# guanlongzhao/fac-via-ppg

Measured on AMD Instinct MI355X. Metric: 22.05 kHz audio samples/sec end-to-end PPG→wav; real-time factor at batch=1, higher is better.
Workload: dtype f32

## Files before the change

fac-via-ppg_amd/csrc/facppg_gemm.hip:

```cpp
#include "facppg_gemm.h"

namespace facppg {
namespace {

constexpr int TN = 64, KCH = 64;

__global__ void k_pack_a(const float* __restrict__ src, float4* __restrict__ dst, int M, int Cin, int taps, int KG, long sm,
                         long sc, long st, long off) {
  const int idx = blockIdx.x * blockDim.x + threadIdx.x;
  const int MB = (M + 31) / 32;
  if (idx >= MB * (KG + 1) * 64) return;
  const int lane = idx & 63, g = (idx >> 6) % (KG + 1), mb = (idx >> 6) / (KG + 1);
  const int m = mb * 32 + (lane & 31), K = Cin * taps;
  float v[4];
  for (int s = 0; s < 4; ++s) {
    const int k = 8 * g + 4 * (lane >> 5) + s;
    const int tap = k / Cin, c = k - tap * Cin;
    v[s] = (m < M && k < K && g < KG) ? src[off + m * sm + c * sc + tap * st] : 0.0f;
  }
  dst[idx] = make_float4(v[0], v[1], v[2], v[3]);
}

struct KArgs {
  GemmArgs g;
  int KG;
  int sk;
};

__device__ __forceinline__ void gemm_epilogue(const GemmArgs& p, int b, int m, int n, float v) {
  if (p.bias) v += p.bias[m];
  if (p.scale) v = v * p.scale[m] + p.shift[m];
  if (p.act == ACT_RELU) v = fmaxf(v, 0.0f);
  else if (p.act == ACT_TANH) v = tanhf(v);
  else if (p.act == ACT_LOG_CLAMP) v = logf(fmaxf(v, 1e-5f));
  if (p.mask) v = v * (float)p.mask[(size_t)b * p.mask_bs + (size_t)m * p.ldmask + n] * 2.0f;
  if (p.res) v += p.res[(size_t)b * p.res_bs + (size_t)m * p.ldres + n];
  if (p.gate_ts) {
    const float T = p.gate_ts[(size_t)b * p.gate_bs + (size_t)m * p.ldgate + n];
    const float S = p.gate_ts[(size_t)b * p.gate_bs + (size_t)(p.M + m) * p.ldgate + n];
    p.C[(size_t)b * p.c_bs + (size_t)m * p.ldc + n] = v * S * (1.0f - T * T);
    p.C[(size_t)b * p.c_bs + (size_t)(p.M + m) * p.ldc + n] = v * T * S * (1.0f - S);
  } else if (p.c_transposed) p.C[(size_t)b * p.c_bs + (size_t)n * p.ldc + m] = v;
  else p.C[(size_t)b * p.c_bs + (size_t)m * p.ldc + n] = v;
}

__global__ __launch_bounds__(256) void k_gemm(KArgs ka) {
  const GemmArgs& p = ka.g;
  __shared__ __attribute__((aligned(16))) float smem[2 * KCH * TN];
  const int tid = threadIdx.x, lane = tid & 63, w = tid >> 6, li = lane & 31, kh = lane >> 5;
  const int b = blockIdx.z / ka.sk, ks = blockIdx.z % ka.sk, n0 = p.col0 + blockIdx.x * TN;
  const int Nb = p.n_valid ? min(p.N, p.n_valid[b] * p.n_valid_mul + p.n_valid_add) : p.N;
  if (n0 >= Nb) return;
  if (p.skip && *p.skip) return;
  const int Ns = p.src_hi > 0 ? (p.n_valid ? min(p.src_hi, p.n_valid[b] * p.n_valid_mul + p.n_valid_add) : p.src_hi) : Nb;
  const int mb = blockIdx.y * 4 + w;
  const int MB = (p.M + 31) / 32;
  const bool active = mb < MB;
  const int K = p.Cin * p.taps;
  const int nch_all = ka.KG / 8;
  const int c_lo = ks * nch_all / ka.sk, c_hi = (ks + 1) * nch_all / ka.sk;

  f32x16 acc[2];
#pragma unroll
  for (int r = 0; r < 16; ++r) { acc[0][r] = 0.0f; acc[1][r] = 0.0f; }

  const float* xb = p.X + (size_t)b * p.x_bs;
  const int col = n0 + lane;
  float stg[16];
  auto stage_load = [&](int c) {
#pragma unroll
    for (int j = 0; j < 16; ++j) {
      const int kk = c * KCH + w * 16 + j;
      const int tap = kk / p.Cin, ch = kk - tap * p.Cin;
      const int sc = col + (tap - p.pad) * p.dil;
      stg[j] = (kk < K && sc >= 0 && sc < Ns) ? xb[(size_t)ch * p.ldx + sc] : 0.0f;
    }
  };
  auto stage_write = [&](int buf) {
    float* dst = smem + buf * (KCH * TN) + (w * 16) * TN + lane;
#pragma unroll
    for (int j = 0; j < 16; ++j) dst[j * TN] = stg[j];
  };

  const float4* ap = p.A + (size_t)(active ? mb : 0) * (ka.KG + 1) * 64 + lane;
  constexpr int RING = 4;
  float4 ar[RING];
  stage_load(c_lo);
#pragma unroll
  for (int i = 0; i < RING - 1; ++i) ar[i] = ap[(size_t)(c_lo * 8 + i) * 64];
  stage_write(c_lo & 1);
  __syncthreads();
  for (int c = c_lo; c < c_hi; ++c) {
    stage_load(c + 1 < c_hi ? c + 1 : c);
    const float* lb = smem + (c & 1) * (KCH * TN) + (4 * kh) * TN + li;
    const int G = c * 8;
#pragma unroll
    for (int g = 0; g < 8; ++g) {
      ar[(g + RING - 1) % RING] = ap[(size_t)(G + g + RING - 1) * 64];
      __builtin_amdgcn_sched_barrier(0);
      const float4 a0 = ar[g % RING];
#pragma unroll
      for (int s = 0; s < 4; ++s) {
        const float av = s == 0 ? a0.x : s == 1 ? a0.y : s == 2 ? a0.z : a0.w;
        acc[0] = mfma32x32x2(av, lb[(8 * g + s) * TN], acc[0]);
        acc[1] = mfma32x32x2(av, lb[(8 * g + s) * TN + 32], acc[1]);
      }
    }
    stage_write((c + 1) & 1);
    __syncthreads();
  }
  if (!active) return;
#pragma unroll
  for (int cb = 0; cb < 2; ++cb) {
    const int n = n0 + cb * 32 + li;
    if (n >= Nb) continue;
#pragma unroll
    for (int r = 0; r < 16; ++r) {
      const int m = mb * 32 + 8 * (r >> 2) + (r & 3) + 4 * kh;
      if (m >= p.M) continue;
      if (ka.sk > 1) p.splitk_ws[(((size_t)ks * p.B + b) * p.M + m) * p.N + n] = acc[cb][r];
      else gemm_epilogue(p, b, m, n, acc[cb][r]);
    }
  }
}

__global__ void k_gemm_reduce(KArgs ka) {
  const GemmArgs& p = ka.g;
  const int n = p.col0 + blockIdx.x * blockDim.x + threadIdx.x, m = blockIdx.y, b = blockIdx.z;
  const int Nb = p.n_valid ? min(p.N, p.n_valid[b] * p.n_valid_mul + p.n_valid_add) : p.N;
  if (n >= Nb) return;
  if (p.skip && *p.skip) return;
  float v = 0.0f;
  for (int ks = 0; ks < ka.sk; ++ks) v += p.splitk_ws[(((size_t)ks * p.B + b) * p.M + m) * p.N + n];
  gemm_epilogue(p, b, m, n, v);
}

}

int pack_a_strided(const float* src, int M, int Cin, int taps, long sm, long sc, long st, long off, float4* dst, hipStream_t s) {
  const int KG = gemm_kpad(Cin * taps) / 8;
  const int total = (round_up(M, 32) / 32) * (KG + 1) * 64;
  k_pack_a<<<(total + 255) / 256, 256, 0, s>>>(src, dst, M, Cin, taps, KG, sm, sc, st, off);
  FACPPG_HIP_CHECK(hipGetLastError());
  return FACPPG_OK;
}

int pack_a(const float* src, int M, int Cin, int taps, float4* dst, hipStream_t s) {
  return pack_a_strided(src, M, Cin, taps, (long)Cin * taps, taps, 1, 0, dst, s);
}

int gemm_launch(const GemmArgs& a, hipStream_t s) {
  FACPPG_REQUIRE(a.A && a.X && a.C && a.M > 0 && a.N > 0 && a.Cin > 0 && a.taps > 0 && a.B > 0 && a.col0 >= 0 && a.col0 < a.N, FACPPG_EINVAL,
                 "gemm_launch: bad arguments");
  KArgs ka;
  ka.g = a;
  ka.KG = gemm_kpad(a.Cin * a.taps) / 8;
  ka.sk = 1;
  dim3 grid((a.N - a.col0 + TN - 1) / TN, (round_up(a.M, 32) / 32 + 3) / 4, a.B);
  const int nch = ka.KG / 8;
  if (a.splitk_ws && nch >= 8) {
    const int sk = nch / 4 < 16 ? nch / 4 : 16;
    const size_t need = (size_t)sk * a.B * a.M * a.N * sizeof(float);
    FACPPG_REQUIRE(need <= a.splitk_ws_bytes, FACPPG_EWORKSPACE, "gemm_launch: split-K buffer has %zu bytes, needs %zu",
                   a.splitk_ws_bytes, need);
    ka.sk = sk;
  }
  grid.z = a.B * ka.sk;
  k_gemm<<<grid, 256, 0, s>>>(ka);
  if (ka.sk > 1) k_gemm_reduce<<<dim3((a.N - a.col0 + 255) / 256, a.M, a.B), 256, 0, s>>>(ka);
  FACPPG_HIP_CHECK(hipGetLastError());
  return FACPPG_OK;
}

}
```

fac-via-ppg_amd/csrc/facppg_taco.hip:

```cpp

#include <algorithm>
#include <cstdlib>
#include <cstring>
#include <mutex>
#include <new>

#include "facppg_gemm.h"

using namespace facppg;

struct facppg_taco {
  facppg_taco_config c;
  int device;
  int coop_limit;
  int wall_khz;
  char* arena;
  float4 *pre0, *pre1, *conv[8], *wih;
  float *conv_b[8], *conv_scale[8], *conv_shift[8];
  float *whh_t[2], *lstm_b;
  float4* mem_w;
  float *dp0_t, *dp1_t, *att_t, *att_b, *dec_t, *dec_b, *q_t, *proj_t, *proj_b;
  float *loc_conv, *loc_dense, *v;
  float *att_coop[5], *dec_coop[5];
  int coop_U[5], coop_nwg[5];
// ... 102 lines not shown
  const int slot = tid % ns, ks = tid / ns;
  if (ks >= KS) return;
  const int k0 = (int)((long)ks * K / KS), k1 = (int)((long)(ks + 1) * K / KS);
  const float4* w = reinterpret_cast<const float4*>(WT) + slot;
  float4 acc = make_float4(0.f, 0.f, 0.f, 0.f);
  for (int kb = k0; kb < k1; kb += UB) {
    float4 wv[UB];
#pragma unroll
    for (int u = 0; u < UB; ++u) wv[u] = w[(size_t)min(kb + u, k1 - 1) * ns];
#pragma unroll
    for (int u = 0; u < UB; ++u) {
      const float vk = kb + u < k1 ? v[kb + u] : 0.0f;
      acc.x = fmaf(wv[u].x, vk, acc.x); acc.y = fmaf(wv[u].y, vk, acc.y);
      acc.z = fmaf(wv[u].z, vk, acc.z); acc.w = fmaf(wv[u].w, vk, acc.w);
    }
  }
  reinterpret_cast<float4*>(part)[ks * ns + slot] = acc;
}
template <int NT>
__device__ __forceinline__ int pick_ks(int Rp, int K) {
  int ks = NT / (Rp >> 2);
  if (ks > K) ks = K;
  return ks < 1 ? 1 : ks;
}
__device__ __forceinline__ float part_sum(const float* part, int Rp, int KS, int r) {
  float s = 0.0f;
#pragma unroll 8
  for (int i = 0; i < KS; ++i) s += part[i * Rp + r];
  return s;
}

__global__ __launch_bounds__(NT) void k_bilstm(const float* __restrict__ xproj, const float* __restrict__ whh_t0,
                                               const float* __restrict__ whh_t1, const int* __restrict__ lengths, int Tin, int H,
                                               float* __restrict__ mem_tm , float* __restrict__ mem_cm ) {
  extern __shared__ float sm[];
  const int dir = blockIdx.x, b = blockIdx.y, tid = threadIdx.x;
  const int R = 4 * H;
  float* hv = sm;
  float* cv = hv + H;
  float* part = cv + H;
  const float* WT = dir ? whh_t1 : whh_t0;
  const int len = lengths ? lengths[b] : Tin;
  const int KS = pick_ks<NT>(R, H);
  for (int i = tid; i < H; i += NT) { hv[i] = 0.0f; cv[i] = 0.0f; }
  __syncthreads();
  for (int s = 0; s < len; ++s) {
    const int t = dir ? len - 1 - s : s;
    matvec_part(WT, H, R, KS, hv, part, tid);
    __syncthreads();
    if (tid < H) {
      const float* xp = xproj + ((size_t)b * Tin + t) * (2 * R) + dir * R;
      const float gi = part_sum(part, R, KS, tid) + xp[tid];
      const float gf = part_sum(part, R, KS, H + tid) + xp[H + tid];
      const float gg = part_sum(part, R, KS, 2 * H + tid) + xp[2 * H + tid];
      const float go = part_sum(part, R, KS, 3 * H + tid) + xp[3 * H + tid];
      const float c = sigm(gf) * cv[tid] + sigm(gi) * tanhf(gg);
      const float h = sigm(go) * tanhf(c);
      cv[tid] = c; hv[tid] = h;
      mem_tm[((size_t)b * Tin + t) * (2 * H) + dir * H + tid] = h;
      mem_cm[((size_t)b * 2 * H + dir * H + tid) * Tin + t] = h;
    }
    __syncthreads();
  }
}

__constant__ unsigned long long g_poll_limit_ticks = 0;
__device__ __forceinline__ unsigned long long poll_tag(const unsigned long long* w, unsigned tag) {
  unsigned long long v;
  const unsigned long long limit = g_poll_limit_ticks;
  unsigned long long t0 = 0;
  unsigned spins = 0;
#pragma unroll 1
  do {
    v = __hip_atomic_load(w, __ATOMIC_RELAXED, __HIP_MEMORY_SCOPE_AGENT);
    if ((++spins & 1023u) == 0 && limit) {
      const unsigned long long now = wall_clock64();
      if (!t0) t0 = now;
      else if (now - t0 > limit) __builtin_trap();
    }
  } while ((unsigned)(v >> 32) != tag);
  return v;
}

template <int BU, int BKR>
__global__ __launch_bounds__(NTC) void k_bilstm_coop(const float* __restrict__ xproj, const float* __restrict__ whh_t0,
                                                     const float* __restrict__ whh_t1, const int* __restrict__ lengths, int Tin,
                                                     int H, unsigned long long* __restrict__ xchg ,
                                                     float* __restrict__ mem_tm, float* __restrict__ mem_cm) {
  constexpr int BKP = NTC / (4 * BU);
  __shared__ float hv[BKP * BKR];
  __shared__ float part[BKP][4 * BU];
  __shared__ float gates[4 * BU];
  const int wg = blockIdx.x, dir = blockIdx.y, b = blockIdx.z, tid = threadIdx.x;
  const int R = 4 * H, KR = (H + BKP - 1) / BKP;
  const int r = tid % (4 * BU), kp = tid / (4 * BU);
  const int u = wg * BU + r % BU, row = (r / BU) * H + u;
  const float* WT = dir ? whh_t1 : whh_t0;
  const int len = lengths ? lengths[b] : Tin;
  float w[BKR];
#pragma unroll
  for (int i = 0; i < BKR; ++i) {
    const int k = kp * KR + i;
    w[i] = (i < KR && k < H && u < H) ? WT[(size_t)k * R + row] : 0.0f;
  }
  for (int i = tid; i < BKP * BKR; i += NTC) hv[i] = 0.0f;
  float c = 0.0f;
  unsigned long long* xb = xchg + (size_t)(b * 2 + dir) * 2 * H;
  __syncthreads();
  for (int s = 0; s < len; ++s) {
    const int t = dir ? len - 1 - s : s;
    const float xp = (kp == 0 && u < H) ? xproj[((size_t)b * Tin + t) * (2 * R) + dir * R + row] : 0.0f;
    float acc = 0.0f;
    const float* hk = hv + kp * KR;
#pragma unroll
    for (int i = 0; i < BKR; ++i) acc = fmaf(w[i], hk[i], acc);
    part[kp][r] = acc;
    __syncthreads();
    if (kp == 0) {
      float g = xp;
#pragma unroll
      for (int j = 0; j < BKP; ++j) g += part[j][r];
      gates[r] = g;
    }
    __syncthreads();
    if (tid < BU && wg * BU + tid < H) {
      const float cn = sigm(gates[BU + tid]) * c + sigm(gates[tid]) * tanhf(gates[2 * BU + tid]);
      const float h = sigm(gates[3 * BU + tid]) * tanhf(cn);
      c = cn;
      const int uu = wg * BU + tid;
      __hip_atomic_store(xb + (size_t)((s + 1) & 1) * H + uu, ((unsigned long long)(unsigned)(s + 1) << 32) | __float_as_uint(h),
                         __ATOMIC_RELAXED, __HIP_MEMORY_SCOPE_AGENT);
      mem_tm[((size_t)b * Tin + t) * (2 * H) + dir * H + uu] = h;
      mem_cm[((size_t)b * 2 * H + dir * H + uu) * Tin + t] = h;
    }
    if (s + 1 < len) {
      const unsigned long long* src = xb + (size_t)((s + 1) & 1) * H;
      for (int i = tid; i < H; i += NTC) {
        hv[i] = __uint_as_float((unsigned)poll_tag(src + i, (unsigned)(s + 1)));
      }
    }
    __syncthreads();
  }
}

struct DecArgs {
  const float *dp0_t, *dp1_t, *att_t, *att_b, *dec_t, *dec_b, *q_t, *proj_t, *proj_b, *loc_conv, *loc_dense, *v;
  const float *att_coop, *dec_coop;
  unsigned long long* xchg;
  const float *att_w4, *dec_w4;
  const float *w1p_t, *b1p;
  unsigned long long* xsplit;
  long long* prof;
  const float* memory;
  const float* pm;
  const int* lengths;
  const int* step_limits;
  const uint8_t* masks;
  float* mel;
  float* gate;
  float* align;
  int* out_len;
  int B, Tin, E, P, A, D, AD, NF, NFIL, KSZ, window, max_steps, U;
  int b0;
  float gate_thr;
  int nwk, dbg_flags;
  unsigned long long* melx;
};

__device__ __forceinline__ int dec_step_limit(const DecArgs& p, int b) {
  return p.step_limits ? min(max(p.step_limits[b], 1), p.max_steps) : p.max_steps;
}

struct DecLds {
  float *in_att, *in_dec, *in_proj, *ac, *dc, *xin, *p1, *pq, *part, *feat, *lconv, *ldense, *vv, *wprev, *wcum, *en;
  int KA, KD, KP, ADp, NFp, Pp, G, AD32;
};

__host__ __device__ inline size_t dec_lds_floats(int P, int E, int A, int D, int NF, int AD, int NFIL, int KSZ, int Tin) {
  (void)NFIL;
  const size_t ADp32 = round_up(AD, 32);
  return (size_t)(P + E + A) + (A + E + D) + (D + E) + A + D + round_up(NF, 4) + round_up(P, 4) + ADp32 + 4096 +
         64 * 32 + (size_t)round_up(2 * KSZ, 2) * 32 + 32 * ADp32 + ADp32 + 3 * (size_t)Tin;
}

__device__ __forceinline__ void dec_carve(const DecArgs& p, float* sm, DecLds& L) {
  L.G = 4 * p.A;
  L.KA = p.P + p.E + p.A;
  L.KD = p.A + p.E + p.D;
  L.KP = p.D + p.E;
  L.ADp = round_up(p.AD, 4); L.NFp = round_up(p.NF + 1, 4); L.Pp = round_up(p.P, 4);
  L.AD32 = round_up(p.AD, 32);
  L.in_att = sm;
  L.in_dec = L.in_att + L.KA;
  L.in_proj = L.in_dec + L.KD;
  L.ac = L.in_proj + L.KP;
  L.dc = L.ac + p.A;
  L.xin = L.dc + p.D;
  L.p1 = L.xin + round_up(p.NF, 4);
  L.pq = L.p1 + L.Pp;
  L.part = L.pq + L.AD32;
  L.feat = L.part + 4096;
  L.lconv = L.feat + 64 * 32;
  L.ldense = L.lconv + round_up(2 * p.KSZ, 2) * 32;
  L.vv = L.ldense + 32 * L.AD32;
  L.wprev = L.vv + L.AD32;
  L.wcum = L.wprev + p.Tin;
  L.en = L.wcum + p.Tin;
}

template <int NT>
__device__ __forceinline__ void dec_init(const DecArgs& p, const DecLds& L, float* sm, int tid) {
  for (int i = tid; i < L.KA + L.KD + L.KP + p.A + p.D + round_up(p.NF, 4) + L.Pp + L.AD32; i += NT) sm[i] = 0.0f;
  const int KK = 2 * p.KSZ;
  for (int i = tid; i < round_up(KK, 2) * 32; i += NT) {
    const int kk = i >> 5, f = i & 31;
    L.lconv[i] = (kk < KK && f < p.NFIL) ? p.loc_conv[f * KK + kk] : 0.0f;
  }
  for (int i = tid; i < 32 * L.AD32; i += NT) {
    const int f = i / L.AD32, a = i % L.AD32;
    L.ldense[i] = (f < p.NFIL && a < p.AD) ? p.loc_dense[a * p.NFIL + f] : 0.0f;
  }
  for (int i = tid; i < L.AD32; i += NT) L.vv[i] = i < p.AD ? p.v[i] : 0.0f;
  for (int i = tid; i < 3 * p.Tin; i += NT) L.wprev[i] = 0.0f;
}

// ... 1065 lines not shown
  w.a0 = take((size_t)B * E * Tin * 4);
  w.a1 = take((size_t)B * E * Tin * 4);
  w.xproj = take((size_t)B * Tin * 4 * c.encoder_embedding_dim * 4);
  w.mem_cm = take((size_t)B * c.encoder_embedding_dim * Tin * 4);
  w.mask = take((size_t)2 * B * c.symbols_embedding_dim * Tin);
  w.xchg = take((size_t)B * 2 * 2 * (c.encoder_embedding_dim / 2) * 8);
  const size_t mx = c.encoder_embedding_dim > c.symbols_embedding_dim ? c.encoder_embedding_dim : c.symbols_embedding_dim;
  w.splitk_bytes = (size_t)16 * B * mx * Tin * 4;
  w.splitk = take(w.splitk_bytes);
  w.total = off;
  return w;
}

}

static int taco_check(const facppg_taco_config* c) {
  FACPPG_REQUIRE(c, FACPPG_EINVAL, "config is NULL");
  FACPPG_REQUIRE(c->n_symbols > 0 && c->symbols_embedding_dim > 0 && c->encoder_embedding_dim > 0 && c->encoder_embedding_dim % 2 == 0,
                 FACPPG_EINVAL, "bad encoder dims");
  FACPPG_REQUIRE(c->symbols_embedding_dim == c->encoder_embedding_dim, FACPPG_EUNSUPPORTED,
                 "symbols_embedding_dim must equal encoder_embedding_dim (prenet feeds the conv bank)");
  FACPPG_REQUIRE(c->encoder_n_convolutions >= 0 && c->encoder_n_convolutions <= 8 && c->postnet_n_convolutions >= 2 &&
                     c->postnet_n_convolutions <= 8 && c->encoder_kernel_size % 2 == 1 && c->postnet_kernel_size % 2 == 1,
                 FACPPG_EUNSUPPORTED, "conv stack sizes out of range");
  FACPPG_REQUIRE(c->attention_rnn_dim == c->decoder_rnn_dim && c->attention_rnn_dim % 4 == 0 && 4 * c->attention_rnn_dim <= 4096,
                 FACPPG_EUNSUPPORTED, "attention_rnn_dim must equal decoder_rnn_dim, be a multiple of 4 and <= 1024");
  FACPPG_REQUIRE(c->attention_location_n_filters >= 1 && c->attention_location_n_filters <= 32 && c->attention_dim >= 1 &&
                     c->attention_dim <= 256,
                 FACPPG_EUNSUPPORTED, "attention_location_n_filters must be <= 32 and attention_dim <= 256 (one MFMA pass each)");
  FACPPG_REQUIRE(c->encoder_embedding_dim <= 768 && c->prenet_dim <= NTC && c->attention_dim <= NTC && c->n_acoustic_feat_dims < NTC &&
                     (2 * c->encoder_embedding_dim) % 4 == 0,
                 FACPPG_EUNSUPPORTED, "decoder dims exceed the 512-thread cooperative workgroup");
  FACPPG_REQUIRE(c->attention_location_kernel_size % 2 == 1 && c->attention_location_n_filters > 0, FACPPG_EUNSUPPORTED,
                 "attention_location_kernel_size must be odd");
  return FACPPG_OK;
}

static size_t taco_count(const facppg_taco_config* c) {
  const size_t S = c->symbols_embedding_dim, E = c->encoder_embedding_dim, H = E / 2, K = c->encoder_kernel_size;
  const size_t P = c->prenet_dim, A = c->attention_rnn_dim, D = c->decoder_rnn_dim, AD = c->attention_dim, NF = c->n_acoustic_feat_dims;
  size_t n = S * c->n_symbols + S * S;
  n += (size_t)c->encoder_n_convolutions * (E * E * K + 5 * E);
  n += 2 * (4 * H * E + 4 * H * H + 8 * H);
  n += P * NF + P * P;
  n += 4 * A * (P + E) + 4 * A * A + 8 * A;
  n += AD * A + AD * E + AD + (size_t)c->attention_location_n_filters * 2 * c->attention_location_kernel_size +
       AD * c->attention_location_n_filters;
  n += 4 * D * (A + E) + 4 * D * D + 8 * D;
  n += NF * (D + E) + NF + (D + E) + 1;
  const size_t PE = c->postnet_embedding_dim, PK = c->postnet_kernel_size;
  for (int j = 0; j < c->postnet_n_convolutions; ++j) {
    const size_t ci = j == 0 ? NF : PE, co = j == c->postnet_n_convolutions - 1 ? NF : PE;
    n += co * ci * PK + 5 * co;
  }
  return n;
}

extern "C" size_t facppg_taco_weight_count(const facppg_taco_config* c) {
  if (taco_check(c) != FACPPG_OK) return 0;
  return taco_count(c);
}

extern "C" int facppg_taco_create(const facppg_taco_config* cfg, const float* wsrc, size_t n_floats, int device, void* stream_,
                                  facppg_taco** out) {
  if (int rc = taco_check(cfg)) return rc;
  FACPPG_REQUIRE(wsrc && out, FACPPG_EINVAL, "NULL argument");
  FACPPG_REQUIRE(n_floats == taco_count(cfg), FACPPG_EINVAL, "weight blob has %zu floats, expected %zu", n_floats, taco_count(cfg));
  hipStream_t s = (hipStream_t)stream_;
  FACPPG_HIP_CHECK(hipSetDevice(device));
  int n_cu = 0;
  FACPPG_HIP_CHECK(hipDeviceGetAttribute(&n_cu, hipDeviceAttributeMultiprocessorCount, device));
  facppg_taco* h = new (std::nothrow) facppg_taco();
  FACPPG_REQUIRE(h, FACPPG_EINVAL, "out of host memory");
  struct Guard {
    facppg_taco* h;
    ~Guard() { if (h) { if (h->arena) (void)hipFree(h->arena); delete h; } }
  } guard{h};
  h->c = *cfg; h->device = device;
  {
    int per_cu = 1;
    const struct { const void* fn; size_t lds; } coop_kernels[] = {
        {(const void*)k_decoder_coop, 150 * 1024}, {(const void*)k_decoder_forced<false>, 150 * 1024}, {(const void*)k_decoder_forced<true>, 150 * 1024}, {(const void*)k_decoder_split<1>, 150 * 1024},
        {(const void*)k_decoder_split<2>, 150 * 1024}, {(const void*)k_decoder_split<3>, 150 * 1024},
        {(const void*)k_bilstm_coop<32, 96>, 0}, {(const void*)k_bilstm_coop<64, 152>, 0}};
    for (const auto& k : coop_kernels) {
      int nb = 0;
      if (k.lds) FACPPG_HIP_CHECK(hipFuncSetAttribute(k.fn, hipFuncAttributeMaxDynamicSharedMemorySize, (int)k.lds));
      FACPPG_HIP_CHECK(hipOccupancyMaxActiveBlocksPerMultiprocessor(&nb, k.fn, NTC, k.lds));
      per_cu = std::min(per_cu, nb);
    }
    const int resident = n_cu * per_cu;
    h->coop_limit = resident - resident / 16;
    static std::mutex poll_mu;
    static unsigned long long poll_devices = 0;
    {
      std::lock_guard<std::mutex> lock(poll_mu);
      const bool known = device < 64 && ((poll_devices >> device) & 1ull);
      if (!known) {
        const char* pl = getenv("FACPPG_POLL_LIMIT");
        const double seconds = pl ? strtod(pl, nullptr) : 20.0;
        int khz = 0;
        FACPPG_HIP_CHECK(hipDeviceGetAttribute(&khz, hipDeviceAttributeWallClockRate, device));
        const unsigned long long ticks = seconds > 0 && khz > 0 ? (unsigned long long)(seconds * 1e3 * khz) : 0ull;
        FACPPG_HIP_CHECK(hipMemcpyToSymbol(HIP_SYMBOL(g_poll_limit_ticks), &ticks, sizeof(ticks)));
        if (device < 64) poll_devices |= 1ull << device;
      }
    }
  }
  (void)hipDeviceGetAttribute(&h->wall_khz, hipDeviceAttributeWallClockRate, device);
  const facppg_taco_config& c = *cfg;
  const int S = c.symbols_embedding_dim, E = c.encoder_embedding_dim, H = E / 2, K = c.encoder_kernel_size;
  const int P = c.prenet_dim, A = c.attention_rnn_dim, D = c.decoder_rnn_dim, AD = c.attention_dim, NF = c.n_acoustic_feat_dims;
  const int NFIL = c.attention_location_n_filters, KSZ = c.attention_location_kernel_size;
  const int PE = c.postnet_embedding_dim, PK = c.postnet_kernel_size;
  const int Pp = round_up(P, 4), ADp = round_up(AD, 4), NFp = round_up(NF + 1, 4), G = 4 * A;

  size_t off = 0;
  auto take = [&](size_t bytes) { size_t o = off; off += (bytes + 255) / 256 * 256; return o; };
  struct { size_t pre0, pre1, conv[8], conv_b[8], conv_sc[8], conv_sh[8], wih, whh[2], lstm_b, mem_w, dp0, dp1, att, att_b, dec, dec_b, q,
           proj, proj_b, lc, ld, v, attc[5], decc[5], att4, dec4, w1p, b1p, post[8], post_b[8], post_sc[8], post_sh[8],
           tf_dp0, tf_dp1, tf_attx, tf_proj; } o;
  o.pre0 = take(packed_a_float4s(S, c.n_symbols) * 16);
  o.pre1 = take(packed_a_float4s(S, S) * 16);
  for (int j = 0; j < c.encoder_n_convolutions; ++j) {
    o.conv[j] = take(packed_a_float4s(E, E * K) * 16);
    o.conv_b[j] = take(E * 4); o.conv_sc[j] = take(E * 4); o.conv_sh[j] = take(E * 4);
  }
  o.wih = take(packed_a_float4s(8 * H, E) * 16);
  o.whh[0] = take((size_t)H * 4 * H * 4); o.whh[1] = take((size_t)H * 4 * H * 4);
  o.lstm_b = take((size_t)8 * H * 4);
  o.mem_w = take(packed_a_float4s(AD, E) * 16);
  o.dp0 = take((size_t)NF * Pp * 4); o.dp1 = take((size_t)P * Pp * 4);
  o.att = take((size_t)(P + E + A) * G * 4); o.att_b = take((size_t)G * 4);
  o.dec = take((size_t)(A + E + D) * G * 4); o.dec_b = take((size_t)G * 4);
  o.q = take((size_t)A * ADp * 4);
  o.proj = take((size_t)(D + E) * NFp * 4); o.proj_b = take((size_t)NFp * 4);
  const int CUs[5] = {8, 20, 40, 75, 150};
  for (int v = 0; v < 5; ++v) {
    const int nwg = (A + CUs[v] - 1) / CUs[v];
    o.attc[v] = take((size_t)nwg * (P + E + A) * 4 * CUs[v] * 4); o.decc[v] = take((size_t)nwg * (A + E + D) * 4 * CUs[v] * 4);
  }
  const int nwk = (A + 3) / 4;
  o.att4 = take((size_t)nwk * (P + E + A) * 16 * 4); o.dec4 = take((size_t)nwk * (A + E + D) * 16 * 4);
  o.w1p = take((size_t)(D + E) * Pp * 4); o.b1p = take((size_t)Pp * 4);
  o.lc = take((size_t)NFIL * 2 * KSZ * 4); o.ld = take((size_t)AD * NFIL * 4); o.v = take((size_t)AD * 4);
  for (int j = 0; j < c.postnet_n_convolutions; ++j) {
    const int ci = j == 0 ? NF : PE, co = j == c.postnet_n_convolutions - 1 ? NF : PE;
    o.post[j] = take(packed_a_float4s(co, ci * PK) * 16);
    o.post_b[j] = take(co * 4); o.post_sc[j] = take(co * 4); o.post_sh[j] = take(co * 4);
  }
  o.tf_dp0 = take(packed_a_float4s(P, NF) * 16); o.tf_dp1 = take(packed_a_float4s(P, P) * 16);
  o.tf_attx = take(packed_a_float4s(G, P) * 16); o.tf_proj = take(packed_a_float4s(NF + 1, D + E) * 16);
  if (hipMalloc((void**)&h->arena, off) != hipSuccess) {
    h->arena = nullptr;
    set_error("hipMalloc(%zu) failed", off);
    return FACPPG_EHIP;
  }
  int rc = FACPPG_OK;
  auto F = [&](size_t x) { return (float*)(h->arena + x); };
  auto F4 = [&](size_t x) { return (float4*)(h->arena + x); };
  auto hipok = [&](hipError_t e) { if (e != hipSuccess && !rc) { set_error("HIP error in facppg_taco_create: %s", hipGetErrorString(e)); rc = FACPPG_EHIP; } };
  auto cpy = [&](float* dst, const float* src, size_t n) { hipok(hipMemcpyAsync(dst, src, n * 4, hipMemcpyDeviceToDevice, s)); };
  auto tr = [&](const float* src, float* dst, int R, int Kk, int Rp, int k_off) {
    const int n = Kk * Rp;
    k_transpose_pad<<<(n + 255) / 256, 256, 0, s>>>(src, dst, R, Kk, Rp, k_off);
  };
  auto bn = [&](const float*& src, int n, float* sc, float* sh) {
// ... 74 lines not shown
    const int n = (D + E + 1) * Pp;
    k_fold_prenet<<<(n + 255) / 256, 256, 0, s>>>(h->proj_t, h->proj_b, h->dp0_t, h->w1p_t, h->b1p, D + E, NF, NFp, Pp);
    if (!rc) rc = pack_a_strided(h->proj_t, NF + 1, D + E, 1, 1, NFp, 0, 0, h->tf_proj, s);
  }
  for (int j = 0; j < c.postnet_n_convolutions; ++j) {
    const int ci = j == 0 ? NF : PE, co = j == c.postnet_n_convolutions - 1 ? NF : PE;
    h->post[j] = F4(o.post[j]); h->post_b[j] = F(o.post_b[j]); h->post_scale[j] = F(o.post_sc[j]); h->post_shift[j] = F(o.post_sh[j]);
    if (!rc) rc = pack_a(src, co, ci, PK, h->post[j], s); src += (size_t)co * ci * PK;
    cpy(h->post_b[j], src, co); src += co;
    bn(src, co, h->post_scale[j], h->post_shift[j]);
  }
  hipok(hipGetLastError());
  hipok(hipStreamSynchronize(s));
  if (!rc && (size_t)(src - wsrc) != n_floats) { set_error("internal: consumed %zu of %zu weights", (size_t)(src - wsrc), n_floats); rc = FACPPG_EINVAL; }
  if (rc) return rc;
  guard.h = nullptr;
  *out = h;
  return FACPPG_OK;
}

extern "C" void facppg_taco_destroy(facppg_taco* h) {
  if (!h) return;
  (void)hipFree(h->arena);
  delete h;
}

extern "C" size_t facppg_taco_workspace_bytes(const facppg_taco* h, int B, int Tin) {
  if (!h || B <= 0 || Tin <= 0) return 0;
  return tws_layout(h->c, B, Tin).total;
}

static int taco_encode_impl(const facppg_taco* h, const float* ppg_dev, const int32_t* lengths_dev, const uint8_t* masks_dev,
                            uint64_t seed, int B, int Tin, float* memory_dev, float* pm_dev, void* ws_, size_t ws_bytes,
                            void* stream_, bool padded_batch) {
  FACPPG_REQUIRE(h && ppg_dev && memory_dev && pm_dev && ws_, FACPPG_EINVAL, "NULL argument");
  FACPPG_REQUIRE(B > 0 && Tin > 0 && B <= 65535, FACPPG_EINVAL, "bad B/Tin");
  const facppg_taco_config& c = h->c;
  const TWs w = tws_layout(c, B, Tin);
  FACPPG_REQUIRE(ws_bytes >= w.total, FACPPG_EWORKSPACE, "workspace has %zu bytes, need %zu", ws_bytes, w.total);
  hipStream_t s = (hipStream_t)stream_;
  char* ws = (char*)ws_;
  float* a0 = (float*)(ws + w.a0);
  float* a1 = (float*)(ws + w.a1);
  float* xproj = (float*)(ws + w.xproj);
  float* mem_cm = (float*)(ws + w.mem_cm);
  const int S = c.symbols_embedding_dim, E = c.encoder_embedding_dim, H = E / 2;
  const uint8_t* masks = masks_dev;
  if (!masks) {
    uint8_t* m = (uint8_t*)(ws + w.mask);
    const size_t n = (size_t)2 * B * S * Tin;
    k_random_mask<<<(unsigned)((n + 255) / 256), 256, 0, s>>>(m, n, seed);
    masks = m;
  }
  GemmArgs g;
  g.B = B; g.N = Tin; g.n_valid = padded_batch ? nullptr : lengths_dev;
  g.splitk_ws = (float*)(ws + w.splitk); g.splitk_ws_bytes = w.splitk_bytes;
  g.A = h->pre0; g.M = S; g.Cin = c.n_symbols; g.X = ppg_dev; g.x_bs = (long)c.n_symbols * Tin; g.ldx = Tin; g.act = ACT_RELU;
  g.mask = masks; g.mask_bs = (long)S * Tin; g.ldmask = Tin; g.C = a0; g.c_bs = (long)S * Tin; g.ldc = Tin;
  if (int rc = gemm_launch(g, s)) return rc;
  g.A = h->pre1; g.Cin = S; g.X = a0; g.x_bs = (long)S * Tin; g.mask = masks + (size_t)B * S * Tin; g.C = a1;
  if (int rc = gemm_launch(g, s)) return rc;
  float* cur = a1;
  float* nxt = a0;
  g.mask = nullptr;
  for (int j = 0; j < c.encoder_n_convolutions; ++j) {
    g.A = h->conv[j]; g.M = E; g.Cin = E; g.taps = c.encoder_kernel_size; g.pad = (c.encoder_kernel_size - 1) / 2; g.X = cur;
    g.x_bs = (long)E * Tin; g.bias = h->conv_b[j]; g.scale = h->conv_scale[j]; g.shift = h->conv_shift[j]; g.C = nxt;
    g.c_bs = (long)E * Tin;
    if (int rc = gemm_launch(g, s)) return rc;
    float* t = cur; cur = nxt; nxt = t;
  }
  GemmArgs p;
  p.splitk_ws = g.splitk_ws; p.splitk_ws_bytes = g.splitk_ws_bytes;
  p.B = B; p.N = Tin; p.n_valid = lengths_dev; p.A = h->wih; p.M = 8 * H; p.Cin = E; p.X = cur; p.x_bs = (long)E * Tin; p.ldx = Tin;
  p.bias = h->lstm_b; p.C = xproj; p.c_bs = (long)Tin * 8 * H; p.ldc = 8 * H; p.c_transposed = 1;
  if (int rc = gemm_launch(p, s)) return rc;
  const char* bilstm_mode = getenv("FACPPG_BILSTM_MODE");
  const bool no_coop = bilstm_mode && !strcmp(bilstm_mode, "single");
  const bool fit32 = (long)B * 2 * ((H + 31) / 32) <= h->coop_limit && (H + 3) / 4 <= 96 && !(bilstm_mode && !strcmp(bilstm_mode, "wide"));
  const bool fit64 = (long)B * 2 * ((H + 63) / 64) <= h->coop_limit && (H + 1) / 2 <= 152;
  if (!no_coop && (fit32 || fit64)) {
    unsigned long long* xchg = (unsigned long long*)(ws + w.xchg);
    FACPPG_HIP_CHECK(hipMemsetAsync(xchg, 0, (size_t)B * 2 * 2 * H * 8, s));
    const float *w0 = h->whh_t[0], *w1 = h->whh_t[1];
    const float* xp = xproj;
    int Tin_ = Tin, H_ = H;
    void* args[] = {(void*)&xp, (void*)&w0, (void*)&w1, (void*)&lengths_dev, (void*)&Tin_, (void*)&H_, (void*)&xchg,
                    (void*)&memory_dev, (void*)&mem_cm};
    if (fit32) FACPPG_HIP_CHECK(launch_coop((const void*)k_bilstm_coop<32, 96>, dim3((H + 31) / 32, 2, B), dim3(NTC), args, 0, s));
    else FACPPG_HIP_CHECK(launch_coop((const void*)k_bilstm_coop<64, 152>, dim3((H + 63) / 64, 2, B), dim3(NTC), args, 0, s));
  } else {
    const int KS = NT / H < H ? NT / H : H;
    const size_t smem = (size_t)(2 * H + (KS > 0 ? KS : 1) * 4 * H) * 4;
    k_bilstm<<<dim3(2, B), NT, smem, s>>>(xproj, h->whh_t[0], h->whh_t[1], lengths_dev, Tin, H, memory_dev, mem_cm);
  }
  GemmArgs m;
  m.splitk_ws = g.splitk_ws; m.splitk_ws_bytes = g.splitk_ws_bytes;
  m.B = B; m.N = Tin; m.n_valid = lengths_dev; m.A = h->mem_w; m.M = c.attention_dim; m.Cin = E; m.X = mem_cm; m.x_bs = (long)E * Tin;
  m.ldx = Tin; m.C = pm_dev; m.c_bs = (long)Tin * c.attention_dim; m.ldc = Tin;
  if (int rc = gemm_launch(m, s)) return rc;
  FACPPG_HIP_CHECK(hipGetLastError());
  return FACPPG_OK;
}

extern "C" int facppg_taco_encode(const facppg_taco* h, const float* ppg_dev, const int32_t* lengths_dev, const uint8_t* masks_dev,
                                  uint64_t seed, int B, int Tin, float* memory_dev, float* pm_dev, void* ws_, size_t ws_bytes,
                                  void* stream_) {
  return taco_encode_impl(h, ppg_dev, lengths_dev, masks_dev, seed, B, Tin, memory_dev, pm_dev, ws_, ws_bytes, stream_, false);
}

extern "C" int facppg_taco_encode_padded(const facppg_taco* h, const float* ppg_dev, const int32_t* lengths_dev,
                                         const int32_t* lengths_host, const uint8_t* masks_dev, uint64_t seed, int B, int Tin,
                                         float* memory_dev, float* pm_dev, void* ws_, size_t ws_bytes, void* stream_) {
  FACPPG_REQUIRE(h && memory_dev && pm_dev, FACPPG_EINVAL, "NULL argument");
  FACPPG_REQUIRE(B > 0 && Tin > 0, FACPPG_EINVAL, "bad B/Tin");
  FACPPG_REQUIRE((lengths_dev == nullptr) == (lengths_host == nullptr), FACPPG_EINVAL, "lengths_dev and lengths_host go together");
  for (int b = 0; lengths_host && b < B; ++b) {
    FACPPG_REQUIRE(lengths_host[b] >= 1 && lengths_host[b] <= Tin, FACPPG_EINVAL, "lengths[%d] = %d is outside [1, Tin = %d]", b,
                   lengths_host[b], Tin);
    FACPPG_REQUIRE(b == 0 || lengths_host[b] <= lengths_host[b - 1], FACPPG_EINVAL,
                   "lengths must be sorted in descending order (pack_padded_sequence, model.py:226): lengths[%d] = %d > lengths[%d] = %d",
                   b, lengths_host[b], b - 1, lengths_host[b - 1]);
  }
  hipStream_t s = (hipStream_t)stream_;
  FACPPG_HIP_CHECK(hipMemsetAsync(memory_dev, 0, (size_t)B * Tin * h->c.encoder_embedding_dim * 4, s));
  FACPPG_HIP_CHECK(hipMemsetAsync(pm_dev, 0, (size_t)B * Tin * h->c.attention_dim * 4, s));
  return taco_encode_impl(h, ppg_dev, lengths_dev, masks_dev, seed, B, Tin, memory_dev, pm_dev, ws_, ws_bytes, stream_, true);
}

namespace {
struct DecWs { size_t mask, xchg, prof, xsplit, total; };
DecWs dec_ws(const facppg_taco_config& c, int B, int max_steps) {
  DecWs w;
  size_t off = 0;
  auto take = [&](size_t bytes) { size_t o = off; off += (bytes + 255) / 256 * 256; return o; };
  w.mask = take((size_t)max_steps * 2 * B * c.prenet_dim);
  w.xchg = take((size_t)B * 2 * c.attention_rnn_dim * 8);
  w.prof = take(32 * 8);
  w.xsplit = take((size_t)B * (c.n_acoustic_feat_dims + 1 + 2 * c.prenet_dim + c.attention_rnn_dim + c.encoder_embedding_dim + c.decoder_rnn_dim + 8) * 8);
  w.total = off;
  return w;
}
}

extern "C" int facppg_taco_draw_dropout(const facppg_taco* h, const uint64_t* seeds_dev, int B, int Tin, int max_steps,
                                        uint8_t* enc_masks_dev, uint8_t* dec_masks_dev, void* stream_) {
  FACPPG_REQUIRE(h && seeds_dev, FACPPG_EINVAL, "NULL argument");
  FACPPG_REQUIRE(B > 0 && Tin > 0 && max_steps > 0, FACPPG_EINVAL, "bad B/Tin/max_steps");
  hipStream_t s = (hipStream_t)stream_;
  const int S = h->c.symbols_embedding_dim, P = h->c.prenet_dim;
  if (enc_masks_dev) {
    const size_t n = (size_t)2 * B * S * Tin;
    k_random_mask_enc_utt<<<(unsigned)((n + 255) / 256), 256, 0, s>>>(enc_masks_dev, seeds_dev, B, S, Tin);
  }
  if (dec_masks_dev) {
    const size_t n = (size_t)max_steps * 2 * B * P;
    k_random_mask_dec_utt<<<(unsigned)((n + 255) / 256), 256, 0, s>>>(dec_masks_dev, seeds_dev, B, P, max_steps);
  }
  FACPPG_HIP_CHECK(hipGetLastError());
  return FACPPG_OK;
}

namespace {
__global__ void k_window_mask(const int32_t* __restrict__ lengths, int B, int Tmax, int window, int t, uint8_t* __restrict__ mask) {
  const int b = blockIdx.y;
  int lo, hi;
  attn_window_range(window, t, lengths[b], &lo, &hi);
  for (int q = blockIdx.x * blockDim.x + threadIdx.x; q < Tmax; q += gridDim.x * blockDim.x)
    mask[(size_t)b * Tmax + q] = (q >= lo && q <= hi) ? 0 : 1;
}
}

extern "C" int facppg_attention_window_mask(const int32_t* lengths_dev, int B, int Tmax, int window, int time_step,
// ... 452 lines not shown
```

Baseline: 4.482 million.

## Add latency-oriented small-N GEMM kernel and DPP-fused BiLSTM cooperative step

Adds a GEMM variant for narrow outputs (N ≤ 256) that uses 32-column tiles and a six-deep register/LDS staging ring to hide global load latency, with incremental index arithmetic instead of per-element divides. It also restructures the cooperative BiLSTM step so gate partial sums are reduced across lanes with DPP moves rather than shared-memory partials and an extra barrier, with the hidden-state buffer double-buffered. Both paths are the default, and the older ones remain selectable through environment variables. The risks are lower MFMA reuse for the small tiles and a more complex thread mapping in the recurrence.

```diff
diff --git a/fac-via-ppg_amd/csrc/facppg_gemm.hip b/fac-via-ppg_amd/csrc/facppg_gemm.hip
--- a/fac-via-ppg_amd/csrc/facppg_gemm.hip
+++ b/fac-via-ppg_amd/csrc/facppg_gemm.hip
@@ -1,4 +1,7 @@
 #include "facppg_gemm.h"
+
+#include <cstdlib>
+#include <cstring>
 
 namespace facppg {
 namespace {
@@ -124,6 +127,110 @@
   }
 }
 
+constexpr int LAT_MAX_N = 256, LTN = 32, LAT_D = 6, LAT_RING = 8;
+
+__global__ __launch_bounds__(256) void k_gemm_lat(KArgs ka) {
+  const GemmArgs& p = ka.g;
+  __shared__ float4 smem[LAT_D][(KCH / 4) * LTN];
+  const int tid = threadIdx.x, lane = tid & 63, w = tid >> 6, li = lane & 31, kh = lane >> 5;
+  const int b = blockIdx.z / ka.sk, ks = blockIdx.z % ka.sk, n0 = p.col0 + blockIdx.x * LTN;
+  const int Nb = p.n_valid ? min(p.N, p.n_valid[b] * p.n_valid_mul + p.n_valid_add) : p.N;
+  if (n0 >= Nb) return;
+  if (p.skip && *p.skip) return;
+  const int Ns = p.src_hi > 0 ? (p.n_valid ? min(p.src_hi, p.n_valid[b] * p.n_valid_mul + p.n_valid_add) : p.src_hi) : Nb;
+  const int mb = blockIdx.y * 4 + w;
+  const int MB = (p.M + 31) / 32;
+  const bool active = mb < MB;
+  const int K = p.Cin * p.taps;
+  const int nch_all = ka.KG / 8;
+  const int c_lo = ks * nch_all / ka.sk, c_hi = (ks + 1) * nch_all / ka.sk;
+
+  f32x16 acc;
+#pragma unroll
+  for (int r = 0; r < 16; ++r) acc[r] = 0.0f;
+
+  const float* xb = p.X + (size_t)b * p.x_bs;
+  const int r8 = tid >> 5, col = n0 + li;
+  const int q64 = KCH / p.Cin, r64 = KCH % p.Cin;
+  const unsigned ldx = (unsigned)p.ldx, Nsu = Ns > 0 ? (unsigned)Ns : 0u;
+  int kk0 = c_lo * KCH + r8 * 8, ch0 = kk0 % p.Cin, tsh0 = (kk0 / p.Cin - p.pad) * p.dil;
+  float st[LAT_D][8];
+  unsigned st_ok[LAT_D];
+  auto stage_load = [&](float (&v)[8], unsigned& okm, bool live) {
+    int ch = ch0, tsh = tsh0;
+    okm = 0u;
+    unsigned off = (unsigned)ch * ldx;
+#pragma unroll
+    for (int j = 0; j < 8; ++j) {
+      const unsigned sc = (unsigned)(col + tsh);
+      const bool ok = live && kk0 + j < K && sc < Nsu;
+      v[j] = xb[ok ? off + sc : 0u];
+      okm |= (ok ? 1u : 0u) << j;
+      off += ldx;
+      if (++ch == p.Cin) { ch = 0; off = 0u; tsh += p.dil; }
+    }
+    kk0 += KCH; tsh0 += q64 * p.dil; ch0 += r64;
+    if (ch0 >= p.Cin) { ch0 -= p.Cin; tsh0 += p.dil; }
+  };
+  auto stage_write = [&](const float (&v)[8], unsigned okm, int slot) {
+    float z[8];
+#pragma unroll
+    for (int j = 0; j < 8; ++j) z[j] = (okm >> j) & 1u ? v[j] : 0.0f;
+    float4* dst = smem[slot] + (2 * r8) * LTN + li;
+    dst[0] = make_float4(z[0], z[1], z[2], z[3]);
+    dst[LTN] = make_float4(z[4], z[5], z[6], z[7]);
+  };
+
+  const float4* ap = p.A + (size_t)(active ? mb : 0) * (ka.KG + 1) * 64 + lane;
+  const int g_last = c_hi * 8 - 1;
+  float4 ar[LAT_RING];
+  stage_load(st[0], st_ok[0], true);
+#pragma unroll
+  for (int i = 0; i < LAT_RING - 1; ++i) ar[i] = ap[(size_t)min(c_lo * 8 + i, g_last) * 64];
+#pragma unroll
+  for (int j = 1; j < LAT_D; ++j)
+    stage_load(st[j], st_ok[j], c_lo + j < c_hi);
+  stage_write(st[0], st_ok[0], 0);
+  __syncthreads();
+  auto round = [&](int base) __attribute__((always_inline)) {
+#pragma unroll
+    for (int j = 0; j < LAT_D; ++j) {
+      const int c = base + j;
+      if (c >= c_hi) return;
+      if (c + 1 < c_hi) stage_write(st[(j + 1) % LAT_D], st_ok[(j + 1) % LAT_D], (j + 1) % LAT_D);
+      const float4* lb = smem[j] + kh * LTN + li;
+      const int G = c * 8;
+      float4 bv[8];
+#pragma unroll
+      for (int g = 0; g < 8; ++g) bv[g] = lb[2 * g * LTN];
+#pragma unroll
+      for (int g = 0; g < 8; ++g) {
+        ar[(g + LAT_RING - 1) % LAT_RING] = ap[(size_t)min(G + g + LAT_RING - 1, g_last) * 64];
+        __builtin_amdgcn_sched_barrier(0);
+        const float4 a0 = ar[g % LAT_RING], b0 = bv[g];
+        acc = mfma32x32x2(a0.x, b0.x, acc);
+        acc = mfma32x32x2(a0.y, b0.y, acc);
+        acc = mfma32x32x2(a0.z, b0.z, acc);
+        acc = mfma32x32x2(a0.w, b0.w, acc);
+      }
+      if (c + LAT_D < c_hi) stage_load(st[j], st_ok[j], true);
+      __syncthreads();
+    }
+  };
+  round(c_lo);
+  for (int base = c_lo + LAT_D; base < c_hi; base += LAT_D) round(base);
+  if (!active) return;
+  const int n = n0 + li;
+  if (n >= Nb) return;
+#pragma unroll
+  for (int r = 0; r < 16; ++r) {
+    const int m = mb * 32 + 8 * (r >> 2) + (r & 3) + 4 * kh;
+    if (m >= p.M) continue;
+    if (ka.sk > 1) p.splitk_ws[(((size_t)ks * p.B + b) * p.M + m) * p.N + n] = acc[r];
+    else gemm_epilogue(p, b, m, n, acc[r]);
+  }
+}
+
 __global__ void k_gemm_reduce(KArgs ka) {
   const GemmArgs& p = ka.g;
   const int n = p.col0 + blockIdx.x * blockDim.x + threadIdx.x, m = blockIdx.y, b = blockIdx.z;
@@ -166,7 +273,13 @@
     ka.sk = sk;
   }
   grid.z = a.B * ka.sk;
-  k_gemm<<<grid, 256, 0, s>>>(ka);
+  const char* shape = getenv("FACPPG_GEMM_SHAPE");
+  if (a.N - a.col0 <= LAT_MAX_N && (long)a.Cin * a.ldx + a.N < (1l << 31) && !(shape && !strcmp(shape, "legacy"))) {
+    grid.x = (a.N - a.col0 + LTN - 1) / LTN;
+    k_gemm_lat<<<grid, 256, 0, s>>>(ka);
+  } else {
+    k_gemm<<<grid, 256, 0, s>>>(ka);
+  }
   if (ka.sk > 1) k_gemm_reduce<<<dim3((a.N - a.col0 + 255) / 256, a.M, a.B), 256, 0, s>>>(ka);
   FACPPG_HIP_CHECK(hipGetLastError());
   return FACPPG_OK;
diff --git a/fac-via-ppg_amd/csrc/facppg_taco.hip b/fac-via-ppg_amd/csrc/facppg_taco.hip
--- a/fac-via-ppg_amd/csrc/facppg_taco.hip
+++ b/fac-via-ppg_amd/csrc/facppg_taco.hip
@@ -208,21 +208,31 @@
   return v;
 }
 
+template <int CTRL>
+__device__ __forceinline__ float lane_mov(float v) {
+  return __int_as_float(__builtin_amdgcn_update_dpp(0, __float_as_int(v), CTRL, 0xF, 0xF, true));
+}
+
+struct BilstmCoopArgs {
+  const float *xproj, *whh_t0, *whh_t1;
+  const int* lengths;
+  int Tin, H;
+  unsigned long long* xchg;
+  float *mem_tm, *mem_cm;
+};
+
 template <int BU, int BKR>
-__global__ __launch_bounds__(NTC) void k_bilstm_coop(const float* __restrict__ xproj, const float* __restrict__ whh_t0,
-                                                     const float* __restrict__ whh_t1, const int* __restrict__ lengths, int Tin,
-                                                     int H, unsigned long long* __restrict__ xchg ,
-                                                     float* __restrict__ mem_tm, float* __restrict__ mem_cm) {
+__device__ __forceinline__ void bilstm_coop_legacy(const BilstmCoopArgs& p) {
   constexpr int BKP = NTC / (4 * BU);
   __shared__ float hv[BKP * BKR];
   __shared__ float part[BKP][4 * BU];
   __shared__ float gates[4 * BU];
   const int wg = blockIdx.x, dir = blockIdx.y, b = blockIdx.z, tid = threadIdx.x;
-  const int R = 4 * H, KR = (H + BKP - 1) / BKP;
+  const int Tin = p.Tin, H = p.H, R = 4 * H, KR = (H + BKP - 1) / BKP;
   const int r = tid % (4 * BU), kp = tid / (4 * BU);
   const int u = wg * BU + r % BU, row = (r / BU) * H + u;
-  const float* WT = dir ? whh_t1 : whh_t0;
-  const int len = lengths ? lengths[b] : Tin;
+  const float* WT = dir ? p.whh_t1 : p.whh_t0;
+  const int len = p.lengths ? p.lengths[b] : Tin;
   float w[BKR];
 #pragma unroll
   for (int i = 0; i < BKR; ++i) {
@@ -231,11 +241,11 @@
   }
   for (int i = tid; i < BKP * BKR; i += NTC) hv[i] = 0.0f;
   float c = 0.0f;
-  unsigned long long* xb = xchg + (size_t)(b * 2 + dir) * 2 * H;
+  unsigned long long* xb = p.xchg + (size_t)(b * 2 + dir) * 2 * H;
   __syncthreads();
   for (int s = 0; s < len; ++s) {
     const int t = dir ? len - 1 - s : s;
-    const float xp = (kp == 0 && u < H) ? xproj[((size_t)b * Tin + t) * (2 * R) + dir * R + row] : 0.0f;
+    const float xp = (kp == 0 && u < H) ? p.xproj[((size_t)b * Tin + t) * (2 * R) + dir * R + row] : 0.0f;
     float acc = 0.0f;
     const float* hk = hv + kp * KR;
 #pragma unroll
@@ -256,8 +266,8 @@
       const int uu = wg * BU + tid;
       __hip_atomic_store(xb + (size_t)((s + 1) & 1) * H + uu, ((unsigned long long)(unsigned)(s + 1) << 32) | __float_as_uint(h),
                          __ATOMIC_RELAXED, __HIP_MEMORY_SCOPE_AGENT);
-      mem_tm[((size_t)b * Tin + t) * (2 * H) + dir * H + uu] = h;
-      mem_cm[((size_t)b * 2 * H + dir * H + uu) * Tin + t] = h;
+      p.mem_tm[((size_t)b * Tin + t) * (2 * H) + dir * H + uu] = h;
+      p.mem_cm[((size_t)b * 2 * H + dir * H + uu) * Tin + t] = h;
     }
     if (s + 1 < len) {
       const unsigned long long* src = xb + (size_t)((s + 1) & 1) * H;
@@ -267,6 +277,98 @@
     }
     __syncthreads();
   }
+}
+
+template <int BU, int BKR, int NB>
+__device__ __forceinline__ void bilstm_coop_steps(const BilstmCoopArgs& p, const float (&w)[BKR], float (*hv)[(NTC / (4 * BU)) * (BKR + 4)],
+                                                  int u, int row, int kp, bool head, int hslot, int len) {
+  constexpr int BKP = NTC / (4 * BU), HVS = BKR + 4;
+  const int dir = blockIdx.y, b = blockIdx.z, tid = threadIdx.x;
+  const int Tin = p.Tin, H = p.H, R = 4 * H;
+  unsigned long long* xb = p.xchg + (size_t)(b * 2 + dir) * 2 * H;
+  float c = 0.0f;
+  for (int s = 0; s < len; ++s) {
+    const int t = dir ? len - 1 - s : s;
+    const float xp = (kp == 0 && u < H) ? p.xproj[((size_t)b * Tin + t) * (2 * R) + dir * R + row] : 0.0f;
+    const float4* hk = reinterpret_cast<const float4*>(hv[s & 1] + kp * HVS);
+    constexpr int CH = 8, NC = (NB + CH - 1) / CH;
+    float4 hb[2][CH];
+#pragma unroll
+    for (int i = 0; i < CH; ++i)
+      if (i < NB) hb[0][i] = hk[i];
+    float acc = 0.0f;
+#pragma unroll
+    for (int ch = 0; ch < NC; ++ch) {
+#pragma unroll
+      for (int i = 0; i < CH; ++i)
+        if ((ch + 1) * CH + i < NB) hb[(ch + 1) & 1][i] = hk[(ch + 1) * CH + i];
+      __builtin_amdgcn_sched_barrier(0);
+#pragma unroll
+      for (int i = 0; i < CH; ++i) {
+        const int j = ch * CH + i;
+        if (j < NB) {
+          const float4 h4 = hb[ch & 1][i];
+          acc = fmaf(w[4 * j], h4.x, acc); acc = fmaf(w[4 * j + 1], h4.y, acc);
+          acc = fmaf(w[4 * j + 2], h4.z, acc); acc = fmaf(w[4 * j + 3], h4.w, acc);
+        }
+      }
+    }
+    float g = xp;
+    if constexpr (BKP == 4) {
+      g += lane_mov<0x00>(acc); g += lane_mov<0x55>(acc); g += lane_mov<0xAA>(acc); g += lane_mov<0xFF>(acc);
+    } else {
+      g += lane_mov<0xA0>(acc); g += lane_mov<0xF5>(acc);
+    }
+    const float gf = lane_mov<0x100 + BKP>(g), gg = lane_mov<0x100 + 2 * BKP>(g), go = lane_mov<0x100 + 3 * BKP>(g);
+    if (head) {
+      const float cn = sigm(gf) * c + sigm(g) * tanhf(gg);
+      const float h = sigm(go) * tanhf(cn);
+      c = cn;
+      __hip_atomic_store(xb + (size_t)((s + 1) & 1) * H + u, ((unsigned long long)(unsigned)(s + 1) << 32) | __float_as_uint(h),
+                         __ATOMIC_RELAXED, __HIP_MEMORY_SCOPE_AGENT);
+      p.mem_tm[((size_t)b * Tin + t) * (2 * H) + dir * H + u] = h;
+      p.mem_cm[((size_t)b * 2 * H + dir * H + u) * Tin + t] = h;
+    }
+    if (s + 1 < len && tid < H)
+      hv[(s + 1) & 1][hslot] = __uint_as_float((unsigned)poll_tag(xb + (size_t)((s + 1) & 1) * H + tid, (unsigned)(s + 1)));
+    __syncthreads();
+  }
+}
+template <int BU, int BKR, int NB>
+__device__ __forceinline__ void bilstm_coop_dispatch(int nb, const BilstmCoopArgs& p, const float (&w)[BKR],
+                                                     float (*hv)[(NTC / (4 * BU)) * (BKR + 4)], int u, int row, int kp, bool head,
+                                                     int hslot, int len) {
+  if (nb == NB) bilstm_coop_steps<BU, BKR, NB>(p, w, hv, u, row, kp, head, hslot, len);
+  else if constexpr (NB > 1) bilstm_coop_dispatch<BU, BKR, NB - 1>(nb, p, w, hv, u, row, kp, head, hslot, len);
+}
+
+template <int BU, int BKR>
+__device__ __forceinline__ void bilstm_coop_fused(const BilstmCoopArgs& p) {
+  constexpr int BKP = NTC / (4 * BU), HVS = BKR + 4, UW = 16 / BKP;
+  static_assert(BKP * 4 * BU == NTC && (BKP == 2 || BKP == 4) && BKR % 4 == 0 && BKP * BKR <= NTC, "bilstm_coop_fused: thread map");
+  __shared__ __attribute__((aligned(16))) float hv[2][BKP * HVS];
+  const int wg = blockIdx.x, dir = blockIdx.y, b = blockIdx.z, tid = threadIdx.x, lane = tid & 63;
+  const int H = p.H, R = 4 * H, KR = (H + BKP - 1) / BKP;
+  const int kp = lane % BKP, gate = (lane / BKP) & 3;
+  const int u = wg * BU + (tid >> 6) * UW + lane / (4 * BKP), row = gate * H + u;
+  const float* WT = dir ? p.whh_t1 : p.whh_t0;
+  const int len = p.lengths ? p.lengths[b] : p.Tin;
+  float w[BKR];
+#pragma unroll
+  for (int i = 0; i < BKR; ++i) {
+    const int k = kp * KR + i;
+    w[i] = (i < KR && k < H && u < H) ? WT[(size_t)k * R + row] : 0.0f;
+  }
+  for (int i = tid; i < 2 * BKP * HVS; i += NTC) (&hv[0][0])[i] = 0.0f;
+  const int hslot = tid < H ? (tid / KR) * HVS + tid % KR : 0;
+  __syncthreads();
+  bilstm_coop_dispatch<BU, BKR, BKR / 4>((KR + 3) / 4, p, w, hv, u, row, kp, lane % (4 * BKP) == 0 && u < H, hslot, len);
+}
+
+template <int BU, int BKR, bool FUSED>
+__global__ __launch_bounds__(NTC) void k_bilstm_coop(BilstmCoopArgs p) {
+  if constexpr (FUSED) bilstm_coop_fused<BU, BKR>(p);
+  else bilstm_coop_legacy<BU, BKR>(p);
 }
 
 struct DecArgs {
@@ -1498,7 +1600,8 @@
     const struct { const void* fn; size_t lds; } coop_kernels[] = {
         {(const void*)k_decoder_coop, 150 * 1024}, {(const void*)k_decoder_forced<false>, 150 * 1024}, {(const void*)k_decoder_forced<true>, 150 * 1024}, {(const void*)k_decoder_split<1>, 150 * 1024},
         {(const void*)k_decoder_split<2>, 150 * 1024}, {(const void*)k_decoder_split<3>, 150 * 1024},
-        {(const void*)k_bilstm_coop<32, 96>, 0}, {(const void*)k_bilstm_coop<64, 152>, 0}};
+        {(const void*)k_bilstm_coop<32, 96, true>, 0}, {(const void*)k_bilstm_coop<64, 152, true>, 0},
+        {(const void*)k_bilstm_coop<32, 96, false>, 0}, {(const void*)k_bilstm_coop<64, 152, false>, 0}};
     for (const auto& k : coop_kernels) {
       int nb = 0;
       if (k.lds) FACPPG_HIP_CHECK(hipFuncSetAttribute(k.fn, hipFuncAttributeMaxDynamicSharedMemorySize, (int)k.lds));
@@ -1739,13 +1842,13 @@
   if (!no_coop && (fit32 || fit64)) {
     unsigned long long* xchg = (unsigned long long*)(ws + w.xchg);
     FACPPG_HIP_CHECK(hipMemsetAsync(xchg, 0, (size_t)B * 2 * 2 * H * 8, s));
-    const float *w0 = h->whh_t[0], *w1 = h->whh_t[1];
-    const float* xp = xproj;
-    int Tin_ = Tin, H_ = H;
-    void* args[] = {(void*)&xp, (void*)&w0, (void*)&w1, (void*)&lengths_dev, (void*)&Tin_, (void*)&H_, (void*)&xchg,
-                    (void*)&memory_dev, (void*)&mem_cm};
-    if (fit32) FACPPG_HIP_CHECK(launch_coop((const void*)k_bilstm_coop<32, 96>, dim3((H + 31) / 32, 2, B), dim3(NTC), args, 0, s));
-    else FACPPG_HIP_CHECK(launch_coop((const void*)k_bilstm_coop<64, 152>, dim3((H + 63) / 64, 2, B), dim3(NTC), args, 0, s));
+    const char* step_env = getenv("FACPPG_BILSTM_STEP");
+    const bool legacy = step_env && !strcmp(step_env, "legacy");
+    BilstmCoopArgs ba{xproj, h->whh_t[0], h->whh_t[1], lengths_dev, Tin, H, xchg, memory_dev, mem_cm};
+    void* args[] = {(void*)&ba};
+    const void* fn = fit32 ? (legacy ? (const void*)k_bilstm_coop<32, 96, false> : (const void*)k_bilstm_coop<32, 96, true>)
+                           : (legacy ? (const void*)k_bilstm_coop<64, 152, false> : (const void*)k_bilstm_coop<64, 152, true>);
+    FACPPG_HIP_CHECK(launch_coop(fn, fit32 ? dim3((H + 31) / 32, 2, B) : dim3((H + 63) / 64, 2, B), dim3(NTC), args, 0, s));
   } else {
     const int KS = NT / H < H ? NT / H : H;
     const size_t smem = (size_t)(2 * H + (KS > 0 ? KS : 1) * 4 * H) * 4;
```

New measurement: 4.620 million, median of 6. 1.03x the previous value.
